# Ladme/groan_rs

Measured on AMD Instinct MI355X. Metric: frames/sec RMSD-fit, 1e6 atoms triclinic, 1/2/4/8 GPUs; HBM GB/s vs peak, higher is better.
Workload: dtype f32 (fp64 accumulators)

## Files before the change

### groan_rs_amd/csrc/gr_api.hip

```cpp
#include <hip/hip_runtime.h>

#include <cmath>
#include <cstdio>
#include <cstdlib>
#include <cstring>
#include <map>
#include <string>
#include <vector>

#include "../../include/groan_hip.h"
#include "gr_container.h"
#include "gr_kernels.h"
#include "gr_hot.h"
#include "gr_resident.h"
#include "gr_small.h"
#include "gr_xtc.h"
#include "gr_shape.h"
#include "gr_xtc_dev.h"
#include "gr_xtc_enc_dev.h"
#include "gr_trr.h"
#include "gr_cellgrid.h"
#include "gr_textio.h"
#include "gr_pool.h"
#include <set>
// ... 91 lines not shown
    uint32_t res_checkin = 0, res_closed = 0;
    uint32_t res_late_seen[2] = { 0, 0 };
    uint64_t res_lean_segments = 0, res_sync_fallbacks = 0;
    GrShapeSet *shape_set_dev = nullptr;
    unsigned long long *shape_mask_dev = nullptr, *shape_mask_host = nullptr; size_t shape_mask_cap = 0;
    uint32_t res_epoch = 0;
    bool res_in_use = false;
    uint64_t res_launches = 0, res_handshake_misses = 0, res_aborts = 0, res_redone_frames = 0;
    GrFrameState *state_dev = nullptr;
    GrFrameState *state_host = nullptr;
    GrFrameState *small_state = nullptr, *small_state_dev = nullptr;
    uint32_t *small_flag = nullptr, *small_flag_dev = nullptr;
    uint32_t small_seq = 0;
    uint32_t small_max = GR_SMALL_MAX_DEFAULT;
    uint64_t small_calls = 0, small_sync_fallbacks = 0;
    uint32_t *bad_dev = nullptr;
    uint32_t *bad_host = nullptr;
    float *pd_out = nullptr; size_t pd_cap = 0;
    hipEvent_t ev0 = nullptr, ev1 = nullptr;
    hipEvent_t pev[6 * GR_MAX_BATCH] = {};
    uint32_t sub_batch = 256;
    uint32_t chunks = 0;
    uint32_t fit_wgs = 0;
    int profile = 0;
    double prof_ms[4] = { 0, 0, 0, 0 };
    uint64_t prof_launches[4] = { 0, 0, 0, 0 };
    uint64_t prof_frames[4] = { 0, 0, 0, 0 };
    uint32_t n_cus = 0;
    unsigned char *xtc_host[2] = { nullptr, nullptr }, *xtc_dev[2] = { nullptr, nullptr }; size_t xtc_host_cap[2] = { 0, 0 }, xtc_dev_cap[2] = { 0, 0 };
    hipEvent_t xtc_ev[2] = { nullptr, nullptr };
    hipEvent_t xtc_unpacked[2] = { nullptr, nullptr };
    hipStream_t unpack_stream = nullptr;
    uint32_t xtc_bank = 0;
    float *wr_host = nullptr; size_t wr_cap = 0;
    void *xe_dev[6] = { nullptr, nullptr, nullptr, nullptr, nullptr, nullptr }; size_t xe_cap[6] = { 0, 0, 0, 0, 0, 0 };
    unsigned char *xe_host[2] = { nullptr, nullptr }; size_t xe_host_cap[2] = { 0, 0 };
    int xtc_dev_encode = 1;
    uint64_t xtc_dev_frames = 0;
    int strict = 0;
    gr_rmsd_plan *in_flight = nullptr;
    uint32_t in_flight_s0 = 0, in_flight_n = 0;
    uint64_t epoch = 1;
    std::string err;
    uint64_t err_index = 0;
    uint64_t counts[2] = { 0, 0 };
};

struct Pending {
    bool active = false, any_ok = false, consistent = true, fused = false, resident = false, rmsd_fast = false;
    uint32_t res_metro_ns = 0; bool res_metro_auto = false;
    uint32_t s0 = 0, nb = 0, n_prof_groups = 0, res_stream = 0, res_streams = 1;
    int fit = 0;
    std::vector<int> pre;
    std::vector<uint64_t> pre_idx;
    std::vector<std::string> pre_msg;
    GrSel sel = {};
    uint64_t group_n = 0;
    bool has_group = false;
    bool small = false; uint32_t small_seq = 0;
    uint32_t res_seq = 0, res_epoch = 0; bool res_fresh = false;
#ifdef GR_EXP_TIMELINE
    unsigned long long *tl_dev = nullptr;
#endif
};

struct gr_rmsd_plan {
    gr_ctx *target = nullptr;
    Pending pend;
    std::string group;
    uint64_t n_ref = 0;
    float *p_dev = nullptr, *w_dev = nullptr;
    float *p_span_dev = nullptr;
    std::vector<grc::Block> ref_blocks;
    bool span_ok = false;
    std::vector<float> w_host;
    GrPlanDev dev = {};
    int exact = 0;
    bool fit_behind_small = false;
    uint32_t last_fallbacks = 0;
    bool resolved = false;
    uint64_t resolved_epoch = 0;
};

namespace {

thread_local std::string g_create_err;

#define HIPCHK(ctx, call)                                                                      \
    do {                                                                                       \
        hipError_t e_ = (call);                                                                \
        if (e_ != hipSuccess) {                                                                \
            (ctx)->err = std::string(#call) + ": " + hipGetErrorString(e_);                    \
            return GR_E_HIP;                                                                   \
        }                                                                                      \
    } while (0)

int fail(gr_ctx *c, int status, const std::string &msg, uint64_t index = 0) {
    c->err = msg; c->err_index = index; return status;
}

GrSel make_sel(const Group &g) {
    GrSel s;
    s.n = (uint32_t)g.n; s.contiguous = g.contiguous ? 1u : 0u; s.start = g.start; s.g0 = g.start >> 8; s.idx = g.idx_dev;
    s.masked = (g.masked && g.mask_dev) ? (g.walk_rw ? 3u : 1u) : 0u; s.span = g.contiguous ? (uint32_t)g.n : g.span; s.mask = g.mask_dev;
    return s;
}

uint32_t chunks_for(const GrSel &s) {
// ... 275 lines not shown

int fetch_states(gr_ctx *c, uint32_t n) {
    HIPCHK(c, hipMemcpyAsync(c->state_host, c->state_dev, n * sizeof(GrFrameState), hipMemcpyDeviceToHost, c->stream));
    HIPCHK(c, hipStreamSynchronize(c->stream));
    return GR_OK;
}

int frame_status(gr_ctx *c, const GrFrameState &st) {
    if (st.status == GR_OK) return GR_OK;
    if (st.status == GR_E_NO_POSITION) return fail(c, GR_E_NO_POSITION, "atom has no position", st.err_index);
    if (st.status == GR_E_NO_MASS) return fail(c, GR_E_NO_MASS, "atom has no mass", st.err_index);
    return fail(c, st.status, "frame analysis failed");
}

static bool small_ok(const gr_ctx *c, const GrSel &sel) { return c->small_max != 0 && c->small_state != nullptr && sel.n <= c->small_max && !c->profile; }
static int small_wait(gr_ctx *c, uint32_t seq, uint32_t words = 1) {
    volatile uint32_t *w = c->small_flag;
    const auto t0 = std::chrono::steady_clock::now();
    for (uint32_t spins = 0; w[0] != seq || w[words - 1] != seq; ++spins) {
        if ((spins & 1023u) == 1023u && std::chrono::steady_clock::now() - t0 > std::chrono::milliseconds(20)) {
            c->small_sync_fallbacks++;
            HIPCHK(c, hipStreamSynchronize(c->stream));
            if (w[0] != seq || w[words - 1] != seq) return fail(c, GR_E_HIP, "a single-wave kernel ended without publishing its result");
            break;
        }
    }
    std::atomic_thread_fence(std::memory_order_acquire);
    c->small_calls++;
    return GR_OK;
}

static int res_next_epoch(gr_ctx *c, uint32_t *epoch) {
    if (++c->res_epoch == 0u) {
        HIPCHK(c, hipStreamSynchronize(c->stream));
        if (c->res_wgrec) HIPCHK(c, hipMemset(c->res_wgrec, 0, c->res_wgrec_cap * sizeof(unsigned long long)));
        HIPCHK(c, hipMemset(c->res_rec, 0, (size_t)GR_MAX_BATCH * 16 * sizeof(unsigned long long)));
        HIPCHK(c, hipMemset(c->res_abort + 2, 0, 2 * sizeof(uint32_t)));
        c->res_epoch = 1u;
    }
    *epoch = c->res_epoch;
    return GR_OK;
}
static int res_test_no_start(gr_ctx *c, uint32_t epoch) {
    if (!c->res_test_no_start) return GR_OK;
    const unsigned long long two = 2ull | ((unsigned long long)epoch << 32);
    c->res_test_no_start = 0;
    HIPCHK(c, hipMemcpyAsync(c->res_abort + 2, &two, sizeof two, hipMemcpyHostToDevice, c->stream));
    HIPCHK(c, hipStreamSynchronize(c->stream));
    return GR_OK;
}
template <int MODE>
static int res_close(gr_ctx *c, uint32_t nb, const double *fit_partials, uint32_t nparts, double sum_w, uint32_t epoch, bool fresh, uint32_t *seq) {
    const uint32_t sq = c->res_seq + 1u;
    k_res_close<MODE><<<dim3(nb), dim3(64), 0, c->stream>>>(fit_partials, nparts, sum_w, c->state_dev, c->res_rec, epoch, fresh ? 1u : 0u, c->res_abort, c->res_closed + nb,
                                                        c->res_out_dev->st, c->res_out_dev->words, &c->res_out_dev->seq, sq);
    HIPCHK(c, hipGetLastError());
    c->res_seq = sq; c->res_closed += nb; *seq = sq;
    return GR_OK;
}
static int res_collect(gr_ctx *c, uint32_t seq, uint32_t nb, uint32_t epoch, bool *started) {
    volatile uint32_t *w = &c->res_out->seq;
    const auto t0 = std::chrono::steady_clock::now();
    for (uint32_t spins = 0; *w != seq; ++spins) {
        if ((spins & 1023u) == 1023u && std::chrono::steady_clock::now() - t0 > std::chrono::milliseconds(20)) {
            c->res_sync_fallbacks++;
            HIPCHK(c, hipStreamSynchronize(c->stream));
            if (*w != seq) return fail(c, GR_E_HIP, "the kernel behind the resident pass ended without publishing its results");
            break;
        }
    }
    std::atomic_thread_fence(std::memory_order_acquire);
    memcpy(c->state_host, c->res_out->st, (size_t)nb * sizeof(GrFrameState));
    memcpy(c->res_words_host, c->res_out->words, 12 * sizeof(uint32_t));
    for (int k = 0; k < 2; ++k) { const uint32_t v = c->res_words_host[8 + k]; c->res_words_host[8 + k] = v - c->res_late_seen[k]; c->res_late_seen[k] = v; }
    *started = c->res_words_host[2] == 1u && c->res_words_host[3] == epoch;
    if (!*started || c->res_words_host[0]) HIPCHK(c, hipStreamSynchronize(c->stream));
    return GR_OK;
}

int center_stage(gr_ctx *c, uint32_t first_slot, uint32_t nf, const GrSel &sel, int kind, int weighted,
                 int mass_first, int target, int only_status = 0) {
    if (small_ok(c, sel)) {
        k_center_small_stage<<<dim3(nf), dim3(64), 0, c->stream>>>(c->frames, c->frame_stride, first_slot, c->masses, sel, c->boxes_dev, kind, weighted, mass_first, target, c->state_dev, only_status);
        HIPCHK(c, hipGetLastError());
        return GR_OK;
    }
    uint32_t nch = chunks_for(sel);
    if (nf > 1 && nch >= 8) nch &= ~7u;
    const dim3 grid(nch, nf), wg(GR_WG);
    if (kind == 0) k_center_sums<0><<<grid, wg, 0, c->stream>>>(c->frames, c->frame_stride, first_slot, c->masses, sel, c->boxes_dev, c->state_dev, weighted, c->cen_partials, only_status);
    else if (kind == 1) k_center_sums<1><<<grid, wg, 0, c->stream>>>(c->frames, c->frame_stride, first_slot, c->masses, sel, c->boxes_dev, c->state_dev, weighted, c->cen_partials, only_status);
    else k_center_sums<2><<<grid, wg, 0, c->stream>>>(c->frames, c->frame_stride, first_slot, c->masses, sel, c->boxes_dev, c->state_dev, weighted, c->cen_partials, only_status);
    k_center_finalize<<<dim3(nf), dim3(GR_WG), 0, c->stream>>>(c->cen_partials, nch, c->boxes_dev, first_slot, kind, weighted, mass_first, target, sel.n, c->state_dev, only_status);
    HIPCHK(c, hipGetLastError());
    return GR_OK;
}

int pbc_center_stages(gr_ctx *c, uint32_t first_slot, uint32_t nf, const GrSel &sel, int weighted, int only_status = 0) {
    if (small_ok(c, sel) && only_status == 0) {
        k_center_small_pbc<<<dim3(nf), dim3(64), 0, c->stream>>>(c->frames, c->frame_stride, first_slot, c->masses, sel, c->boxes_dev, weighted, c->state_dev);
        HIPCHK(c, hipGetLastError());
        return GR_OK;
    }
    int st = center_stage(c, first_slot, nf, sel, 1, 0, 0, 0, only_status);
    if (st != GR_OK) return st;
    return center_stage(c, first_slot, nf, sel, 2, weighted, 0, 1, only_status);
}

static bool center_onepass_ok(const gr_ctx *c, const GrSel &sel) {
    return c->com_onepass_min != 0 && (sel.contiguous || sel.masked) && sel.n >= c->com_onepass_min && c->two_pass;
// ... 1349 lines not shown
int gr_ctx_set_tuning(gr_ctx *c, int key, int64_t value) try {
    if (!c) return GR_E_INVALID_ARG;
    { int st = busy_check(c); if (st) return st; }
    switch (key) {
    case GR_TUNE_SUB_BATCH: if (value < 1 || value > GR_MAX_BATCH) break; c->sub_batch = (uint32_t)value; return GR_OK;
    case GR_TUNE_CHUNKS: if (value < 0 || value > GR_MAX_CHUNKS) break; c->chunks = (uint32_t)value; return GR_OK;
    case GR_TUNE_FIT_WGS: if (value < 0 || value > 65535) break; c->fit_wgs = (uint32_t)value; return GR_OK;
    case GR_TUNE_FUSE: c->fuse = value ? 1 : 0; return GR_OK;
    case GR_TUNE_SMALL_CALLS: if (value < 0 || value > 65536) break; c->small_max = (uint32_t)value; return GR_OK;
    case GR_TUNE_TWO_PASS: c->two_pass = value ? 1 : 0; return GR_OK;
    case GR_TUNE_RESIDENT: if (value < 0 || value > 2) break; c->resident = value; return GR_OK;
    case GR_TUNE_MASKED_SELECTIONS: if (value != 0 && value != 1) break; c->masked_sel = (int)value; return GR_OK;
    case GR_TUNE_XTC_DEVICE_ENCODE: if (value != 0 && value != 1) break; c->xtc_dev_encode = (int)value; return GR_OK;
    case GR_TUNE_RMSD_FAST: if (value != 0 && value != 1) break; c->rmsd_fast = (int)value; return GR_OK;
    case GR_TUNE_RMSD_FAST_MIN: if (value < 0 || value > 0x7fffffff) break; c->rmsd_fast_min = (uint32_t)value; return GR_OK;
    case GR_TUNE_RMSD_FAST_SIGMAS: if (value < 0 || value > 1000) break; c->rmsd_fast_sigmas = (int)value; return GR_OK;
    case GR_TUNE_PAIRDIST_SYMMETRIC: if (value != 0 && value != 1) break; c->pd_sym = (int)value; return GR_OK;
    case GR_TUNE_RESIDENT_WG_GROUPS: if (value != 0 && (value < 64 || value > GR_RES_GROUPS || value % 64 != 0)) break; c->res_wg_groups = (int)value; return GR_OK;
    case GR_TUNE_RESIDENT_STREAMS: if (value < 0 || value > GR_RES_MAX_STREAMS) break; c->res_streams = (int)value; return GR_OK;
    case GR_TUNE_RESIDENT_METRO_NS: if (value < 0 || value > 1000000 || (value > 1 && value < 100)) break; c->res_metro_ns = (int)value; c->metro = gr_ctx::Metro(); return GR_OK;
    case GR_TUNE_RESIDENT_FIT_LAST: if (value < 0 || value > 2) break; c->res_fit_last = (int)value; return GR_OK;
    case GR_TUNE_STREAM_WGS_PER_CU: if (value < 0 || value > 8) break; c->stream_wgs_cu = (int)value; return GR_OK;
    case GR_TUNE_CENTER_RESIDENT: if (value < 0 || value > 1) break; c->center_resident = (int)value; return GR_OK;
    case GR_TUNE_TRANSLATE_ROWS: if (value < 0 || value > 1) break; c->translate_rows = (int)value; return GR_OK;
    case GR_TUNE_RESIDENT_FILL: if (value < 1 || value > 16) break; c->res_fill16 = (int)value; return GR_OK;
    case GR_TUNE_RESIDENT_GROUPS: if (value != 2) break; return GR_OK;
    case GR_TUNE_TEST_RESIDENT_NO_START: c->res_test_no_start = value ? 1 : 0; return GR_OK;
    case GR_TUNE_TEST_RESIDENT_ABORT_AT: c->res_test_abort_at = value < 0 ? 0xFFFFFFFFu : (uint32_t)value; return GR_OK;
    default: break;
    }
    return fail(c, GR_E_INVALID_ARG, "unknown tuning key or value out of range");
} catch (...) { return gr_abi_guard(); }

static int rmsd_exact(gr_rmsd_plan *p, gr_ctx *c, const GrSel &sel, uint32_t first_slot, uint32_t nf, int fit) {
    int st = pbc_center_stages(c, first_slot, nf, sel, 1); if (st) return st;
    if (small_ok(c, sel)) {
        k_rmsd_small<1><<<dim3(nf), dim3(64), 0, c->stream>>>(c->frames, c->frame_stride, first_slot, c->masses, sel, c->boxes_dev, p->dev, c->state_dev, 1, nullptr, nullptr, 0u);
    } else {
        const uint32_t nch = chunks_for(sel);
        k_rmsd_accum<1><<<dim3(nch, nf), dim3(GR_WG), 0, c->stream>>>(c->frames, c->frame_stride, first_slot, c->masses, sel, c->boxes_dev, p->dev, c->state_dev, c->acc_partials);
        k_rmsd_finalize<1><<<dim3(nf), dim3(GR_WG), 0, c->stream>>>(c->acc_partials, nch, c->frames, c->frame_stride, first_slot, sel, c->boxes_dev, p->dev, c->state_dev);
    }
    if (fit) {
        const uint32_t gx = (uint32_t)std::min<uint64_t>(((c->n >> 2) + GR_WG * 4 - 1) / (GR_WG * 4) + 1, 1024);
        k_fit_pk<false><<<dim3(gx, nf), dim3(GR_WG), 0, c->stream>>>(c->frames, c->frame_stride, first_slot, (uint32_t)c->n, c->boxes_dev, p->dev, c->state_dev, c->masses, sel, nullptr);
    }
    HIPCHK(c, hipGetLastError());
    return GR_OK;
}

static int segment_begin(gr_rmsd_plan *p, uint32_t s0, uint32_t nb, int fit) {
    gr_ctx *c = p->target;
    Pending &q = p->pend;
    q = Pending();
    q.s0 = s0; q.nb = nb; q.fit = fit; q.active = true;
    SlotUse use(c, s0, nb);
    const Group *g = find_group(c, p->group.c_str());
    q.pre.assign(nb, GR_OK); q.pre_idx.assign(nb, 0); q.pre_msg.assign(nb, std::string());
    for (uint32_t f = 0; f < nb; ++f) {
        int s = box_check(c, s0 + f);
        if (s == GR_OK && !g) s = fail(c, GR_E_GROUP_NOT_FOUND, p->group);
        if (s == GR_OK && g->n == 0) s = fail(c, GR_E_EMPTY_GROUP, p->group);
        q.pre[f] = s;
        if (s != GR_OK) { q.pre_msg[f] = c->err; q.pre_idx[f] = c->err_index; }
        q.any_ok = q.any_ok || s == GR_OK;
    }
    if (!q.any_ok) return GR_OK;
    const GrSel sel = make_sel(*g);
    q.sel = sel; q.group_n = g->n; q.has_group = true;
    if (!p->resolved || p->resolved_epoch != c->epoch) {
        p->resolved_epoch = c->epoch;
        bool same = (g->n == p->n_ref);
        if (same) { size_t k = 0; for (uint64_t i : grc::expand(g->blocks)) { const float a = c->masses_host[i], b = p->w_host[k++]; if (!(a == b)) { same = false; break; } } }
        p->dev.w_is_mass = same ? 1u : 0u; p->resolved = true;
        p->span_ok = p->p_span_dev != nullptr && g->masked && g->mask_dev != nullptr && g->blocks == p->ref_blocks;
    }
    q.consistent = (g->n == p->n_ref);
    const bool fast_asked = c->two_pass && c->rmsd_fast && p->dev.w_is_mass != 0 && g->n >= c->rmsd_fast_min && ((!fit && sel.contiguous) || (sel.masked && p->span_ok));
    const bool small = q.consistent && !p->exact && small_ok(c, sel) && !fast_asked;
    if (small && nb == 1) {
        q.small = true; q.small_seq = ++c->small_seq;
        k_rmsd_small<0><<<dim3(1), dim3(64), 0, c->stream>>>(c->frames, c->frame_stride, s0, c->masses, sel, c->boxes_dev, p->dev,
                                                         c->state_dev, 0, c->small_state_dev, c->small_flag_dev, q.small_seq);
        if (fit) k_fit_pk<false><<<dim3(fit_grid(c, 1), 1), dim3(GR_WG), 0, c->stream>>>(c->frames, c->frame_stride, s0, (uint32_t)c->n, c->boxes_dev, p->dev, c->state_dev, c->masses, sel, nullptr);
        p->fit_behind_small = fit != 0;
        HIPCHK(c, hipGetLastError());
        return GR_OK;
    }
    bool states_unset = false;
    {
        bool all_ok = true;
        for (uint32_t f = 0; f < nb; ++f) all_ok = all_ok && q.pre[f] == GR_OK;
        states_unset = all_ok;
        if (!all_ok) {
            for (uint32_t f = 0; f < nb; ++f) { GrFrameState z = {}; z.err_index = GR_NOIDX; z.status = q.pre[f]; c->state_host[f] = z; }
            HIPCHK(c, hipMemcpyAsync(c->state_dev, c->state_host, nb * sizeof(GrFrameState), hipMemcpyHostToDevice, c->stream));
        }
    }
    auto zero_states = [&]() -> int { if (!states_unset) return GR_OK; states_unset = false; return state_reset(c, nb); };
    int st;
    if (!(q.consistent && !p->exact && !small)) { st = zero_states(); if (st) return st; }
    if (small) {
        k_rmsd_small<0><<<dim3(nb), dim3(64), 0, c->stream>>>(c->frames, c->frame_stride, s0, c->masses, sel, c->boxes_dev, p->dev, c->state_dev, 1, nullptr, nullptr, 0u);
        if (fit) k_fit_pk<false><<<dim3(fit_grid(c, nb), nb), dim3(GR_WG), 0, c->stream>>>(c->frames, c->frame_stride, s0, (uint32_t)c->n, c->boxes_dev, p->dev, c->state_dev, c->masses, sel, nullptr);
        HIPCHK(c, hipGetLastError());
    } else if (!q.consistent) {
        st = pbc_center_stages(c, s0, nb, sel, 1); if (st) return st;
    } else if (p->exact) {
        st = rmsd_exact(p, c, sel, s0, nb, fit); if (st) return st;
    } else {
        const uint32_t sb = c->sub_batch;
        const bool lite = fit && sel.contiguous && c->two_pass;
        const bool msk = sel.masked && p->span_ok;
        const bool fast = c->two_pass && c->rmsd_fast && p->dev.w_is_mass != 0 && g->n >= c->rmsd_fast_min && ((!fit && sel.contiguous) || msk);
        q.rmsd_fast = fast;
        p->dev.fast_sigmas = (float)c->rmsd_fast_sigmas;
        GrPlanDev plan_span = p->dev; plan_span.p = p->p_span_dev;
        const uint32_t n_groups = (nb + sb - 1) / sb;
        if (lite) {
            size_t need = 0;
            for (uint32_t f0 = 0; f0 < nb; f0 += sb) need = std::max(need, (size_t)nb * fit_grid(c, std::min<uint32_t>(sb, nb - f0)) * (GR_WG / 64));
            if (need > c->fit_partials_cap) {
                if (c->fit_partials) (void)hipFree(c->fit_partials);
                c->fit_partials = nullptr; c->fit_partials_cap = 0;
                HIPCHK(c, hipMalloc(&c->fit_partials, need * sizeof(double)));
                c->fit_partials_cap = need;
            }
        }
        const bool fused = (lite || fast) && c->fuse;
        q.fused = fused;
        hipStream_t S = c->stream;
        uint32_t res_streams = 1, res_gwg = GR_RES_GROUPS;
        const bool res_msk = fit && msk && c->two_pass && p->dev.w_is_mass != 0;
        uint32_t res_wgs = resident_wgs(c, lite || res_msk, nb, sel, &res_streams, &res_gwg);
        if (res_wgs && !resident_acquire(c->device)) res_wgs = 0;
        if (res_wgs) c->res_in_use = true;
        if (res_wgs) {
            const uint32_t res_stream = res_wgs * res_streams;
            const uint32_t n_fin = std::min<uint32_t>(res_streams > 8 ? GR_RES_MAX_FIN : 8, c->res_max_wgs - res_stream);
            if ((size_t)nb * res_wgs * GrResShape::WAVES > c->fit_partials_cap) {
                if (c->fit_partials) (void)hipFree(c->fit_partials);
                c->fit_partials = nullptr; c->fit_partials_cap = 0;
                HIPCHK(c, hipMalloc(&c->fit_partials, (size_t)nb * res_wgs * GrResShape::WAVES * sizeof(double)));
                c->fit_partials_cap = (size_t)nb * res_wgs * GrResShape::WAVES;
            }
            const size_t rec_words = (size_t)nb * ((res_wgs + GR_RES_REC_PAD - 1u) & ~(uint32_t)(GR_RES_REC_PAD - 1u)) * GR_RES_REC_WORDS;
            if (rec_words > c->res_wgrec_cap) {
                if (c->res_wgrec) (void)hipFree(c->res_wgrec);
                c->res_wgrec = nullptr; c->res_wgrec_cap = 0;
                HIPCHK(c, hipMalloc(&c->res_wgrec, rec_words * sizeof(unsigned long long)));
                HIPCHK(c, hipMemsetAsync(c->res_wgrec, 0, rec_words * sizeof(unsigned long long), S));
                c->res_wgrec_cap = rec_words;
            }
            GrResCtl ctl;
            st = res_next_epoch(c, &ctl.epoch); if (st) return st;
            ctl.wgrec = c->res_wgrec; ctl.rec = c->res_rec; ctl.abort = c->res_abort; ctl.progress = c->res_progress; ctl.n_stream = res_stream; ctl.n_fin = n_fin;
            ctl.checkin_target = c->res_checkin + res_stream + n_fin; ctl.fresh_states = states_unset ? 1u : 0u;
            ctl.wgs_frame = res_wgs; ctl.streams = res_streams; ctl.groups_wg = res_gwg;
            ctl.team_waves = resident_team_waves(res_wgs, res_streams);
            ctl.patience_ticks = (unsigned long long)c->wall_khz * 3000ull; ctl.start_ticks = (unsigned long long)c->wall_khz * 200ull;
            ctl.test_abort_frame = c->res_test_abort_at; c->res_test_abort_at = 0xFFFFFFFFu;
            {
                const uint64_t shape = ((uint64_t)res_wgs << 40) ^ ((uint64_t)res_streams << 32) ^ ((uint64_t)res_gwg << 16) ^ (uint64_t)(c->n & 0xFFFF) ^ ((uint64_t)(sel.start == 0 && sel.n == c->n) << 63);
                uint32_t period_ns = 0;
                q.res_metro_auto = false;
                if (c->res_metro_ns >= 100) period_ns = (uint32_t)c->res_metro_ns;
                else if (c->res_metro_ns == 0) {
                    gr_ctx::Metro &m = c->metro;
                    if (m.shape != shape) { m = gr_ctx::Metro(); m.shape = shape; }
                    if (m.off_for) m.off_for--;
                    else if (m.free_ns > 0) period_ns = (uint32_t)(m.T_ns + 0.5);
                    q.res_metro_auto = true;
                }
                q.res_metro_ns = period_ns;
                ctl.metro_t16 = (uint32_t)std::min<uint64_t>(0xFFFFFFFFull, (uint64_t)period_ns * (uint64_t)c->wall_khz * 16ull / 1000000ull);
                ctl.metro_lead = (uint32_t)((uint64_t)c->wall_khz * 2000ull / 1000000ull);
            }
#ifdef GR_EXP_STEPTIME
            {
                static unsigned long long *dbg_dev = nullptr;
                if (!dbg_dev) (void)hipMalloc(&dbg_dev, (size_t)GR_MAX_CHUNKS * 8 * 4 * sizeof(unsigned long long));
                ctl.dbg = getenv("GR_STEPTIME") ? dbg_dev : nullptr;
                g_steptime_dbg = ctl.dbg;
            }
#endif
#ifdef GR_EXP_TIMELINE
            {
                static unsigned long long *tl_dev = nullptr; static size_t tl_cap = 0;
                if (nb > tl_cap) { if (tl_dev) (void)hipFree(tl_dev); tl_dev = nullptr; tl_cap = 0; if (hipMalloc(&tl_dev, (size_t)nb * 8 * sizeof(unsigned long long)) == hipSuccess) tl_cap = nb; }
                ctl.tl = getenv("GR_TIMELINE") ? tl_dev : nullptr;
                if (ctl.tl) HIPCHK(c, hipMemsetAsync(ctl.tl, 0, (size_t)nb * 8 * sizeof(unsigned long long), S));
                q.tl_dev = ctl.tl;
            }
#endif
            float *frames = c->frames; size_t stride = c->frame_stride; uint32_t slot0 = s0, nfr = nb, natoms = (uint32_t)c->n;
            const float *masses = c->masses; GrSel sel_arg = sel; const GrBox *boxes = c->boxes_dev; GrPlanDev plan = res_msk ? plan_span : p->dev;
            GrFrameState *states = c->state_dev; double *fparts = c->fit_partials;
            void *args[] = { &frames, &stride, &slot0, &nfr, &natoms, &masses, &sel_arg, &boxes, &plan, &states, &fparts, &ctl };
            bool ubox = true;
            for (uint32_t f = 1; f < nb && ubox; ++f) ubox = memcmp(&c->boxes_host[s0 + f], &c->boxes_host[s0], sizeof(GrBox)) == 0;
#ifdef GR_EXP_NO_UBOX
            ubox = false;
#endif
            const bool whole = sel.start == 0 && sel.n == c->n;
            const bool fit_last = c->res_fit_last ? c->res_fit_last == 2 : (uint64_t)res_stream * 10u >= (uint64_t)c->res_max_wgs * 9u;
            const void *fn = resident_fn(p->dev.w_is_mass != 0, ubox, whole, fit_last);
            const uint32_t lanes = GrResShape::LANES, lds = GrResShape::LDS_BYTES;
            st = res_test_no_start(c, ctl.epoch); if (st) return st;
            if (c->profile) EVREC(c, c->pev[0], true, S);
            const hipError_t le = hipLaunchKernel(fn, dim3(res_stream + n_fin), dim3(lanes), args, lds, S);
            if (le == hipSuccess) {
                if (c->profile) EVREC(c, c->pev[1], true, S);
                c->res_checkin += res_stream + n_fin;
                q.res_fresh = states_unset; q.res_epoch = ctl.epoch;
                states_unset = false;
                st = res_close<0>(c, nb, c->fit_partials, res_wgs * GrResShape::WAVES, p->dev.sw, ctl.epoch, q.res_fresh, &q.res_seq); if (st) return st;
                q.resident = true; q.res_stream = res_stream; q.res_streams = res_streams;
                q.rmsd_fast = false;
                c->res_last_streams = res_streams;
            } else {
                (void)hipGetLastError();
                c->res_max_wgs = 0;
                resident_done(c);
            }
        }
        if (!q.resident) { st = zero_states(); if (st) return st; }
        for (uint32_t g = 0; g < n_groups && !q.resident; ++g) {
            const uint32_t f0 = g * sb, nf = std::min<uint32_t>(sb, nb - f0), nch = batch_chunks(c, sel, nf), gx = fit_grid(c, nf);
            GrAccPartial *parts = c->acc_partials + (size_t)f0 * GR_MAX_CHUNKS;
            if (c->profile) EVREC(c, c->pev[6 * g], true, S);
            if (lite) k_sums_pk<false><<<dim3(nch, nf), dim3(GR_WG), 0, S>>>(c->frames, c->frame_stride, s0 + f0, c->masses, sel, c->boxes_dev, p->dev, parts,
                                                                             fused ? c->fuse_cnt + f0 : nullptr, c->state_dev + f0);
            else if (fast && msk) k_sums_pk<false, true, true><<<dim3(nch, nf), dim3(GR_WG), 0, S>>>(c->frames, c->frame_stride, s0 + f0, c->masses, sel, c->boxes_dev, plan_span, parts,
                                                                                                      fused ? c->fuse_cnt + f0 : nullptr, c->state_dev + f0);
            else if (fast) k_sums_pk<false, true><<<dim3(nch, nf), dim3(GR_WG), 0, S>>>(c->frames, c->frame_stride, s0 + f0, c->masses, sel, c->boxes_dev, p->dev, parts,
                                                                                        fused ? c->fuse_cnt + f0 : nullptr, c->state_dev + f0);
            else k_rmsd_accum<0><<<dim3(nch, nf), dim3(GR_WG), 0, S>>>(c->frames, c->frame_stride, s0 + f0, c->masses, sel, c->boxes_dev, p->dev, c->state_dev + f0, parts);
            if (c->profile) EVREC(c, c->pev[6 * g + 1], true, S);
            if (!fused) {
                if (c->profile) EVREC(c, c->pev[6 * g + 2], true, S);
                if (lite) k_rmsd_finalize_lite<false><<<dim3(nf), dim3(64), 0, S>>>(parts, nch, c->frames, c->frame_stride, s0 + f0, sel, c->boxes_dev, p->dev, c->state_dev + f0);
                else if (fast) k_rmsd_finalize_lite<false, true><<<dim3(nf), dim3(64), 0, S>>>(parts, nch, c->frames, c->frame_stride, s0 + f0, sel, c->boxes_dev, msk ? plan_span : p->dev, c->state_dev + f0);
                else k_rmsd_finalize<0><<<dim3(nf), dim3(GR_WG), 0, S>>>(parts, nch, c->frames, c->frame_stride, s0 + f0, sel, c->boxes_dev, p->dev, c->state_dev + f0);
                if (c->profile) EVREC(c, c->pev[6 * g + 3], true, S);
            }
            if (fit) {
                if (c->profile) EVREC(c, c->pev[6 * g + 4], true, S);
                if (lite) k_fit_pk<true><<<dim3(gx, nf), dim3(GR_WG), stream_lds(c, GR_STREAM_WGS_CU_DEFAULT), S>>>(c->frames, c->frame_stride, s0 + f0, (uint32_t)c->n, c->boxes_dev, p->dev, c->state_dev + f0, c->masses, sel, c->fit_partials + (size_t)f0 * gx * (GR_WG / 64));
                else k_fit_pk<false><<<dim3(gx, nf), dim3(GR_WG), 0, S>>>(c->frames, c->frame_stride, s0 + f0, (uint32_t)c->n, c->boxes_dev, p->dev, c->state_dev + f0, c->masses, sel, nullptr);
                if (c->profile) EVREC(c, c->pev[6 * g + 5], true, S);
                if (lite) k_rmsd_close<<<dim3(nf), dim3(64), 0, S>>>(c->fit_partials + (size_t)f0 * gx * (GR_WG / 64), gx * (GR_WG / 64), p->dev.sw, c->state_dev + f0);
            }
        }
        HIPCHK(c, hipGetLastError());
        if (c->profile) q.n_prof_groups = q.resident ? 0 : n_groups;
    }
    if (!q.resident) HIPCHK(c, hipMemcpyAsync(c->state_host, c->state_dev, nb * sizeof(GrFrameState), hipMemcpyDeviceToHost, c->stream));
    return GR_OK;
}

static int segment_end(gr_rmsd_plan *p, float *rmsd_out, int *status_out, float *R_out, std::vector<GrFrameState> *final_states = nullptr) {
    gr_ctx *c = p->target;
    Pending &q = p->pend;
    if (!q.active) return fail(c, GR_E_INVALID_ARG, "no batch in flight");
    q.active = false;
    const uint32_t nb = q.nb, s0 = q.s0;
    const int fit = q.fit;
    int first_err = GR_OK; uint64_t first_err_index = 0; std::string first_err_msg; uint64_t first_counts[2] = { 0, 0 };
    auto note = [&](int s) { if (s != GR_OK && first_err == GR_OK) { first_err = s; first_err_index = c->err_index; first_err_msg = c->err; first_counts[0] = c->counts[0]; first_counts[1] = c->counts[1]; } };
    if (!q.any_ok) {
        for (uint32_t f = 0; f < nb; ++f) {
            c->err = q.pre_msg[f]; c->err_index = q.pre_idx[f]; note(q.pre[f]);
            if (status_out) status_out[f] = q.pre[f];
            if (rmsd_out) rmsd_out[f] = NAN;
            if (R_out) for (int k = 0; k < 9; ++k) R_out[9 * (size_t)f + k] = NAN;
        }
        if (final_states) { final_states->assign(nb, GrFrameState{}); for (uint32_t f = 0; f < nb; ++f) { (*final_states)[f].status = q.pre[f]; (*final_states)[f].err_index = GR_NOIDX; } }
    } else {
        if (!q.has_group) return fail(c, GR_E_INVALID_ARG, "batch state lost");
        const GrSel sel = q.sel;
        bool res_started = false;
        if (q.small) { const int sw = small_wait(c, q.small_seq); if (sw) return sw; c->state_host[0] = *c->small_state; }
        else if (q.resident) { const int sw = res_collect(c, q.res_seq, nb, q.res_epoch, &res_started); if (sw) { resident_done(c); return sw; } }
        else HIPCHK(c, hipStreamSynchronize(c->stream));
        std::vector<uint8_t> redo;
        std::vector<uint8_t> torn;
#ifdef GR_EXP_TIMELINE
        if (q.resident && q.tl_dev) {
            std::vector<unsigned long long> tl((size_t)nb * 8);
            if (hipMemcpy(tl.data(), q.tl_dev, tl.size() * sizeof(unsigned long long), hipMemcpyDeviceToHost) == hipSuccess) {
                double sum[8] = { 0 }; double period = 0; uint64_t n = 0, polled = 0, fpolls = 0; unsigned long long prev = 0;
                for (uint32_t f = 0; f < nb; ++f) {
                    const unsigned long long *t = &tl[(size_t)f * 8];
                    if (!t[0] || !t[1] || !t[5] || !(t[6] & 0xFFFFFFFFFFFFull)) continue;
                    const unsigned long long look = t[6] & 0xFFFFFFFFFFFFull;
                    sum[0] += (double)((long long)(t[1] - t[0])); sum[1] += (double)((long long)(t[2] - t[1])); sum[2] += (double)((long long)(t[3] - t[2]));
                    sum[3] += (double)((long long)(t[4] - t[3])); sum[4] += (double)((long long)(t[5] - t[4])); sum[5] += (double)((long long)(look - t[5]));
                    sum[6] += (double)((long long)(look - t[0]));
                    if (prev) period += (double)((long long)(t[0] - prev));
                    prev = t[0];
                    polled += (t[6] >> 48) != 0; fpolls += t[7]; n++;
                }
                if (n > 1) fprintf(stderr, "timeline (%llu frames, us): pub->all records %.2f | ->team totals %.2f | state load %.2f | closing %.2f | publish+store %.2f | ->wg0 looks %.2f | pub->look %.2f | period %.3f | wg0 polled for %.0f %% of the frames | finalizer polls per frame %.1f\n",
                                   (unsigned long long)n, sum[0] / n / 100.0, sum[1] / n / 100.0, sum[2] / n / 100.0, sum[3] / n / 100.0, sum[4] / n / 100.0, sum[5] / n / 100.0, sum[6] / n / 100.0,
                                   period / (n - 1) / 100.0, 100.0 * polled / n, (double)fpolls / n);
            }
        }
#endif
        if (q.resident) {
            resident_done(c);
            if (!res_started) {
                c->res_handshake_misses++;
                c->res_backoff = c->res_backoff ? std::min<uint32_t>(c->res_backoff * 2u, 1024u) : 4u;
                c->res_skip = c->res_backoff + 1u;
                const int fit_again = q.fit;
                const uint32_t s0_again = q.s0, nb_again = q.nb;
                int st2 = segment_begin(p, s0_again, nb_again, fit_again);
                if (st2) { p->pend.active = false; resident_done(c); return st2; }
                return segment_end(p, rmsd_out, status_out, R_out, final_states);
            }
            c->res_backoff = 0;
            if (q.res_fresh) c->res_lean_segments++;
            const uint32_t aborted = c->res_words_host[0];
            if (aborted) {
                (void)hipMemset(c->res_abort, 0, sizeof(uint32_t));
// ... 131 lines not shown
                std::vector<GrFrameState> fs2;
                Pending sub;
                std::swap(sub, p->pend);
                st_redo = segment_begin(p, s0 + f0, f1 - f0, fit);
                if (st_redo == GR_OK) {
                    const int st_nested = segment_end(p, nullptr, nullptr, nullptr, &fs2);
                    if (fs2.size() != (size_t)(f1 - f0)) st_redo = st_nested != GR_OK ? st_nested : GR_E_HIP;
                    else for (uint32_t f = f0; f < f1; ++f) res[f] = fs2[f - f0];
                } else { p->pend.active = false; resident_done(c); }
                std::swap(sub, p->pend);
                c->res_redone_frames += f1 - f0;
                f0 = f1;
            }
            c->resident = keep;
            if (st_redo != GR_OK) return st_redo;
        }
        if (q.rmsd_fast) {
            for (uint32_t f0 = 0; f0 < nb; ) {
                if (res[f0].status != GR_ST_REDO_EXACT) { if (q.pre[f0] == GR_OK) c->rmsd_fast_frames++; ++f0; continue; }
                uint32_t f1 = f0;
                while (f1 < nb && res[f1].status == GR_ST_REDO_EXACT) ++f1;
                const uint32_t nf = f1 - f0, nch = batch_chunks(c, sel, nf);
                SlotUse use(c, s0 + f0, nf);
                int st = state_reset(c, nf); if (st) return st;
                GrAccPartial *parts = c->acc_partials;
                k_rmsd_accum<0><<<dim3(nch, nf), dim3(GR_WG), 0, c->stream>>>(c->frames, c->frame_stride, s0 + f0, c->masses, sel, c->boxes_dev, p->dev, c->state_dev, parts);
                k_rmsd_finalize<0><<<dim3(nf), dim3(GR_WG), 0, c->stream>>>(parts, nch, c->frames, c->frame_stride, s0 + f0, sel, c->boxes_dev, p->dev, c->state_dev);
                if (fit) {
                    const uint32_t gx = fit_grid(c, nf);
                    k_fit_pk<false><<<dim3(gx, nf), dim3(GR_WG), 0, c->stream>>>(c->frames, c->frame_stride, s0 + f0, (uint32_t)c->n, c->boxes_dev, p->dev, c->state_dev, c->masses, sel, nullptr);
                }
                HIPCHK(c, hipGetLastError());
                st = fetch_states(c, nf); if (st) return st;
                for (uint32_t f = f0; f < f1; ++f) res[f] = c->state_host[f - f0];
                c->rmsd_exact_redos += nf;
                f0 = f1;
            }
        }
        for (uint32_t f0 = 0; f0 < nb; ) {
            if (res[f0].status != GR_ST_FALLBACK || (!redo.empty() && redo[f0])) { ++f0; continue; }
            uint32_t f1 = f0;
            while (f1 < nb && res[f1].status == GR_ST_FALLBACK && (redo.empty() || !redo[f1])) ++f1;
            const uint32_t nf = f1 - f0;
            p->last_fallbacks += nf;
            SlotUse use(c, s0 + f0, nf);
            int st = state_reset(c, nf); if (st) return st;
            st = rmsd_exact(p, c, sel, s0 + f0, nf, fit); if (st) return st;
            st = fetch_states(c, nf); if (st) return st;
            for (uint32_t f = f0; f < f1; ++f) res[f] = c->state_host[f - f0];
            f0 = f1;
        }
        for (uint32_t f = 0; f < nb; ++f) {
            int s = res[f].status;
            if (q.pre[f] != GR_OK) { s = q.pre[f]; c->err = q.pre_msg[f]; c->err_index = q.pre_idx[f]; }
            else if (!torn.empty() && torn[f]) s = fail(c, GR_E_HIP, "the resident RMSD-fit pass stalled while this frame was being fitted: some of its atoms carry the fitted coordinates, others the original ones (frame index in gr_last_error_index)", f);
            else if (s == GR_OK && !q.consistent) {
                c->counts[0] = p->n_ref; c->counts[1] = q.group_n;
                s = fail(c, GR_E_INCONSISTENT_GROUP, p->group);
            } else if (s != GR_OK) {
                s = frame_status(c, res[f]);
            }
            note(s);
            if (status_out) status_out[f] = s;
            if (rmsd_out) rmsd_out[f] = (s == GR_OK) ? res[f].rmsd : NAN;
            if (R_out) for (int k = 0; k < 9; ++k) R_out[9 * (size_t)f + k] = (s == GR_OK) ? res[f].R[k] : NAN;
        }
        if (final_states) *final_states = res;
    }
    if (first_err != GR_OK) { c->err = first_err_msg; c->err_index = first_err_index; c->counts[0] = first_counts[0]; c->counts[1] = first_counts[1]; }
    return first_err;
}

static int rmsd_batch_impl(gr_rmsd_plan *p, uint32_t first_slot, uint32_t n_frames, float *rmsd_out, int *status_out, float *R_out, int fit) {
    if (!p || !p->target) return GR_E_INVALID_ARG;
    gr_ctx *c = p->target;
    int st = slot_check(c, first_slot, n_frames); if (st) return st;
    (void)hipSetDevice(c->device);
    if (p->pend.active) return fail(c, GR_E_INVALID_ARG, "a batch begun with gr_rmsd_batch_begin is still in flight");
    p->last_fallbacks = 0;
    int first_err = GR_OK; uint64_t e_idx = 0; std::string e_msg; uint64_t e_cnt[2] = { 0, 0 };
    for (uint32_t b0 = 0; b0 < n_frames; b0 += GR_MAX_BATCH) {
        const uint32_t nb = std::min<uint32_t>(GR_MAX_BATCH, n_frames - b0);
        st = segment_begin(p, first_slot + b0, nb, fit);
        if (st) { p->pend.active = false; resident_done(c); return st; }
        st = segment_end(p, rmsd_out ? rmsd_out + b0 : nullptr, status_out ? status_out + b0 : nullptr, R_out ? R_out + 9 * (size_t)b0 : nullptr);
        if (st == GR_E_HIP) return st;
        if (st != GR_OK && first_err == GR_OK) { first_err = st; e_idx = c->err_index; e_msg = c->err; e_cnt[0] = c->counts[0]; e_cnt[1] = c->counts[1]; }
    }
    if (first_err != GR_OK) { c->err = e_msg; c->err_index = e_idx; c->counts[0] = e_cnt[0]; c->counts[1] = e_cnt[1]; }
    return first_err;
}

int gr_rmsd_batch_begin(gr_rmsd_plan *p, uint32_t first_slot, uint32_t n, int fit) try {
    if (!p || !p->target) return GR_E_INVALID_ARG;
    gr_ctx *c = p->target;
    int st = slot_check(c, first_slot, n); if (st) return st;
    if (n > GR_MAX_BATCH) return fail(c, GR_E_INVALID_ARG, "at most 1024 frames per asynchronous batch");
    if (p->pend.active) return fail(c, GR_E_INVALID_ARG, "a batch is already in flight on this plan");
    (void)hipSetDevice(c->device);
    p->last_fallbacks = 0;
    st = segment_begin(p, first_slot, n, fit ? 1 : 0);
    if (st) { p->pend.active = false; resident_done(c); } else { c->in_flight = p; c->in_flight_s0 = first_slot; c->in_flight_n = n; }
    return st;
} catch (...) { return gr_abi_guard(); }
int gr_rmsd_batch_end(gr_rmsd_plan *p, float *rmsd_out, int *status_out, float *R_out) try {
    if (!p || !p->target) return GR_E_INVALID_ARG;
    (void)hipSetDevice(p->target->device);
// ... 970 lines not shown
```

### groan_rs_amd/csrc/gr_resident.h

```cpp
#pragma once
#include <type_traits>
#include "gr_hot.h"

struct GrResShape {
    static constexpr int LANES = 512, WAVES = LANES / 64;
#ifndef GR_RES_K
#define GR_RES_K 6
#endif
    static constexpr int K = GR_RES_K;
    static constexpr int R = 8;
    static constexpr int PARK_F4 = K * 3 * LANES;
    static constexpr int WSUM_F = R * WAVES * 32;
#ifdef GR_EXP_TIMELINE
    static constexpr int TL_BYTES = 128 * 4 * 8;
#else
    static constexpr int TL_BYTES = 0;
#endif
    static constexpr int LDS_BYTES = PARK_F4 * 16 + WSUM_F * 4 + R * WAVES * 8 + 3 * R * 4 + 2 * WAVES * 4 + TL_BYTES;
    static constexpr int REC_PER_WAVE = 256 / WAVES, LANES_PER_REC = 64 / REC_PER_WAVE, WORDS_PER_LANE = 32 / LANES_PER_REC;
};
#ifndef GR_RES_SLEEP
#define GR_RES_SLEEP 2
#endif
#ifndef GR_RES_BAL
// ... 892 lines not shown
        request(i + 1, nxt);
#endif
        if (i < n_turns) {
            if (MODE == 1) sums_cen(i, cur, Bs);
            else if (V) sums(i, cur, Bs, va, vb);
            lds_put(ps, va);
            if (ps == 0u) { Q0 = vb; asm volatile("; set 0 in"); } else if (ps == 1u) { Q1 = vb; asm volatile("; set 1 in"); } else if (ps == 2u) { Q2 = vb; asm volatile("; set 2 in"); }
            else if (ps == 3u) { Q3 = vb; asm volatile("; set 3 in"); } else if (ps == 4u) { Q4 = vb; asm volatile("; set 4 in"); } else { Q5 = vb; asm volatile("; set 5 in"); }
            if (!V && MODE != 1) sums(i, cur, Bs, va, vb);
        }
#if GR_RES_LATE_COMBINE
        if (i == n_turns && n_turns > 0u && claim(n_turns - 1u)) { if constexpr (MODE == 1) combine_cen(n_turns - 1u); else combine_rmsd(n_turns - 1u); }
#endif
    };
    auto step = [&](uint32_t i, Landing &cur, Landing &nxt) { if constexpr (FL) step_sums_first(i, cur, nxt); else step_fit_first(i, cur, nxt); };
    for (uint32_t i = 0; i < n_iter && !bail; i += 2) {
        step(i, L0, L1);
        if (!bail && i + 1 < n_iter) step(i + 1, L1, L0);
    }
    if (lane == 0) {
        ctl.progress[wg_all * WAVES + wave] = n_fitted;
        (void)__hip_atomic_fetch_max(reinterpret_cast<unsigned long long *>(ctl.abort + 6), (unsigned long long)wall_clock64(), __ATOMIC_RELAXED, __HIP_MEMORY_SCOPE_AGENT);
        if (n_late) (void)__hip_atomic_fetch_add(ctl.abort + 8, n_late, __ATOMIC_RELAXED, __HIP_MEMORY_SCOPE_AGENT);
        if (n_waited) (void)__hip_atomic_fetch_add(ctl.abort + 9, n_waited, __ATOMIC_RELAXED, __HIP_MEMORY_SCOPE_AGENT);
#ifdef GR_EXP_STEPTIME
        if (ctl.dbg) {
            unsigned long long *o = ctl.dbg + (size_t)(wg_all * WAVES + wave) * 4u;
            unsigned long long tot = 0; for (int k = 0; k < 7; ++k) tot += st_acc[k];
            o[0] = st_acc[4]; o[1] = st_acc[7] | (st_combines << 32);
            o[2] = (__builtin_amdgcn_s_getreg((20 << 0) | (0 << 6) | (3 << 11)) & 7u) | (simd_of[wave] << 8);
            o[3] = tot;
        }
        if ((wg_all == 0u || wg_all == ctl.n_stream / 2u) && (wave == 0u || wave == 5u)) {
            unsigned long long *o = reinterpret_cast<unsigned long long *>(ctl.abort + 16) + ((wg_all ? 2u : 0u) + (wave ? 1u : 0u)) * 8u;
            for (int k = 0; k < 8; ++k) o[k] = st_acc[k];
        }
#endif
        if (clk_wave) {
            const unsigned long long dc = (unsigned long long)clock64() - clk_c0, dw = (unsigned long long)wall_clock64() - clk_w0;
            gr_st_agent(ctl.abort + 10, (uint32_t)(dc >> 8)); gr_st_agent(ctl.abort + 11, (uint32_t)(dw >> 8));
        }
    }
#ifdef GR_EXP_TIMELINE
    if (tl_wg && wave == 0 && !bail) {
        for (uint32_t t = (n_turns > 128u ? n_turns - 128u : 0u) + lane; t < n_turns; t += 64u) {
            const size_t f = kf(t);
            ctl.tl[f * 8 + 0] = tls[(t & 127u) * 4u + 0u];
            ctl.tl[f * 8 + 6] = tls[(t & 127u) * 4u + 1u] | (tls[(t & 127u) * 4u + 2u] << 48);
        }
    }
#endif
}

template <int MODE>
__global__ __launch_bounds__(64) void k_res_close(const double *__restrict__ fit_partials, uint32_t nparts, double sum_w, GrFrameState *state,
                                                  const unsigned long long *__restrict__ rec, uint32_t epoch, uint32_t fresh_states, uint32_t *ctl_words,
                                                  uint32_t done_target, GrFrameState *out_states, uint32_t *out_words, uint32_t *out_seq, uint32_t seq) {
    constexpr uint32_t NW = sizeof(GrFrameState) / 4u, W_RMSD = offsetof(GrFrameState, rmsd) / 4u, W_STATUS = offsetof(GrFrameState, status) / 4u;
    static_assert(sizeof(GrFrameState) % 4u == 0 && NW <= 64u, "a frame state is exported by one wave, a word per lane");
    const uint32_t frame = blockIdx.x, lane = threadIdx.x;
    uint32_t *sw = reinterpret_cast<uint32_t *>(state + frame);
    uint32_t w = 0u;
    if (fresh_states && (uint32_t)(gr_ld_agent(rec + (size_t)frame * 16u) >> 32) != epoch) {
        GrFrameState z = {};
        z.err_index = GR_NOIDX; z.status = GR_ST_ABORTED;
        if (lane < NW) { w = reinterpret_cast<const uint32_t *>(&z)[lane]; sw[lane] = w; }
    } else if (lane < NW) w = sw[lane];
    const int status = __shfl((int)w, (int)W_STATUS, 64);
    if (MODE == 0 && status == 0) {
        double s0 = 0.0, s1 = 0.0, s2 = 0.0, s3 = 0.0;
        const double *p = fit_partials + (size_t)frame * nparts;
        uint32_t k = lane;
        for (; k + 192 < nparts; k += 256) { s0 += p[k]; s1 += p[k + 64]; s2 += p[k + 128]; s3 += p[k + 192]; }
        for (; k < nparts; k += 64) s0 += p[k];
        const double s = gr_wave_sum((s0 + s1) + (s2 + s3));
        float r = 0.0f;
        if (lane == 0) { r = (float)sqrt(fmax(s, 0.0) / sum_w); state[frame].rmsd = r; }
        r = __shfl(r, 0, 64);
        if (lane == W_RMSD) w = __float_as_uint(r);
    }
    if (lane < NW) reinterpret_cast<uint32_t *>(out_states + frame)[lane] = w;
    __threadfence_system();
    uint32_t n = 0u;
    if (lane == 0) n = __hip_atomic_fetch_add(ctl_words + 12, 1u, __ATOMIC_ACQ_REL, __HIP_MEMORY_SCOPE_AGENT) + 1u;
    n = (uint32_t)__builtin_amdgcn_readfirstlane((int)n);
    if (n != done_target) return;
    if (lane < 12u) out_words[lane] = gr_ld_agent(ctl_words + lane);
    __threadfence_system();
    if (lane == 0) __hip_atomic_store(out_seq, seq, __ATOMIC_RELEASE, __HIP_MEMORY_SCOPE_SYSTEM);
}
```

Baseline: 140,600.

## Pack eight frames per close workgroup and trim per-segment host bookkeeping

The resident close kernel now handles eight frames per workgroup, one wave per frame. Only wave 0 of each workgroup does the system fence and the completion-counter atomic, so there are fewer system-scope fences and atomics per segment. Host-side setup reuses the Pending vectors, records only the frames that failed, and computes the same-box and all-ok flags in the existing check loop. The cost is a block-wide barrier and explicit waitcnts, plus a lower_bound lookup when reporting per-frame errors.

```diff
diff --git a/groan_rs_amd/csrc/gr_api.hip b/groan_rs_amd/csrc/gr_api.hip
--- a/groan_rs_amd/csrc/gr_api.hip
+++ b/groan_rs_amd/csrc/gr_api.hip
@@ -167,8 +167,15 @@
     uint32_t s0 = 0, nb = 0, n_prof_groups = 0, res_stream = 0, res_streams = 1;
     int fit = 0;
     std::vector<int> pre;
-    std::vector<uint64_t> pre_idx;
-    std::vector<std::string> pre_msg;
+    struct PreFail { uint32_t frame; uint64_t index; std::string msg; };
+    std::vector<PreFail> pre_fail;
+    const PreFail &failed(uint32_t f) const { return *std::lower_bound(pre_fail.begin(), pre_fail.end(), f, [](const PreFail &a, uint32_t b) { return a.frame < b; }); }
+    void restart() {
+        std::vector<int> a; std::vector<PreFail> b;
+        a.swap(pre); b.swap(pre_fail); b.clear();
+        *this = Pending();
+        a.swap(pre); b.swap(pre_fail);
+    }
     GrSel sel = {};
     uint64_t group_n = 0;
     bool has_group = false;
@@ -550,10 +557,11 @@
 template <int MODE>
 static int res_close(gr_ctx *c, uint32_t nb, const double *fit_partials, uint32_t nparts, double sum_w, uint32_t epoch, bool fresh, uint32_t *seq) {
     const uint32_t sq = c->res_seq + 1u;
-    k_res_close<MODE><<<dim3(nb), dim3(64), 0, c->stream>>>(fit_partials, nparts, sum_w, c->state_dev, c->res_rec, epoch, fresh ? 1u : 0u, c->res_abort, c->res_closed + nb,
-                                                        c->res_out_dev->st, c->res_out_dev->words, &c->res_out_dev->seq, sq);
+    const uint32_t wgs = (nb + GR_RES_CLOSE_WAVES - 1u) / GR_RES_CLOSE_WAVES;
+    k_res_close<MODE><<<dim3(wgs), dim3(GR_RES_CLOSE_WAVES * 64), 0, c->stream>>>(fit_partials, nparts, sum_w, c->state_dev, c->res_rec, epoch, fresh ? 1u : 0u, nb, c->res_abort,
+                                                                              c->res_closed + wgs, c->res_out_dev->st, c->res_out_dev->words, &c->res_out_dev->seq, sq);
     HIPCHK(c, hipGetLastError());
-    c->res_seq = sq; c->res_closed += nb; *seq = sq;
+    c->res_seq = sq; c->res_closed += wgs; *seq = sq;
     return GR_OK;
 }
 static int res_collect(gr_ctx *c, uint32_t seq, uint32_t nb, uint32_t epoch, bool *started) {
@@ -2009,18 +2017,20 @@
 static int segment_begin(gr_rmsd_plan *p, uint32_t s0, uint32_t nb, int fit) {
     gr_ctx *c = p->target;
     Pending &q = p->pend;
-    q = Pending();
+    q.restart();
     q.s0 = s0; q.nb = nb; q.fit = fit; q.active = true;
     SlotUse use(c, s0, nb);
     const Group *g = find_group(c, p->group.c_str());
-    q.pre.assign(nb, GR_OK); q.pre_idx.assign(nb, 0); q.pre_msg.assign(nb, std::string());
+    bool all_ok = true, same_box = true;
+    q.pre.resize(nb);
     for (uint32_t f = 0; f < nb; ++f) {
         int s = box_check(c, s0 + f);
         if (s == GR_OK && !g) s = fail(c, GR_E_GROUP_NOT_FOUND, p->group);
         if (s == GR_OK && g->n == 0) s = fail(c, GR_E_EMPTY_GROUP, p->group);
         q.pre[f] = s;
-        if (s != GR_OK) { q.pre_msg[f] = c->err; q.pre_idx[f] = c->err_index; }
-        q.any_ok = q.any_ok || s == GR_OK;
+        if (s != GR_OK) { all_ok = false; q.pre_fail.push_back({ f, c->err_index, c->err }); }
+        else q.any_ok = true;
+        same_box = same_box && memcmp(&c->boxes_host[s0 + f], &c->boxes_host[s0], sizeof(GrBox)) == 0;
     }
     if (!q.any_ok) return GR_OK;
     const GrSel sel = make_sel(*g);
@@ -2046,8 +2056,6 @@
     }
     bool states_unset = false;
     {
-        bool all_ok = true;
-        for (uint32_t f = 0; f < nb; ++f) all_ok = all_ok && q.pre[f] == GR_OK;
         states_unset = all_ok;
         if (!all_ok) {
             for (uint32_t f = 0; f < nb; ++f) { GrFrameState z = {}; z.err_index = GR_NOIDX; z.status = q.pre[f]; c->state_host[f] = z; }
@@ -2154,8 +2162,7 @@
             const float *masses = c->masses; GrSel sel_arg = sel; const GrBox *boxes = c->boxes_dev; GrPlanDev plan = res_msk ? plan_span : p->dev;
             GrFrameState *states = c->state_dev; double *fparts = c->fit_partials;
             void *args[] = { &frames, &stride, &slot0, &nfr, &natoms, &masses, &sel_arg, &boxes, &plan, &states, &fparts, &ctl };
-            bool ubox = true;
-            for (uint32_t f = 1; f < nb && ubox; ++f) ubox = memcmp(&c->boxes_host[s0 + f], &c->boxes_host[s0], sizeof(GrBox)) == 0;
+            bool ubox = same_box;
 #ifdef GR_EXP_NO_UBOX
             ubox = false;
 #endif
@@ -2227,7 +2234,8 @@
     auto note = [&](int s) { if (s != GR_OK && first_err == GR_OK) { first_err = s; first_err_index = c->err_index; first_err_msg = c->err; first_counts[0] = c->counts[0]; first_counts[1] = c->counts[1]; } };
     if (!q.any_ok) {
         for (uint32_t f = 0; f < nb; ++f) {
-            c->err = q.pre_msg[f]; c->err_index = q.pre_idx[f]; note(q.pre[f]);
+            if (q.pre[f] != GR_OK) { const Pending::PreFail &e = q.failed(f); c->err = e.msg; c->err_index = e.index; }
+            note(q.pre[f]);
             if (status_out) status_out[f] = q.pre[f];
             if (rmsd_out) rmsd_out[f] = NAN;
             if (R_out) for (int k = 0; k < 9; ++k) R_out[9 * (size_t)f + k] = NAN;
@@ -2465,7 +2473,7 @@
         }
         for (uint32_t f = 0; f < nb; ++f) {
             int s = res[f].status;
-            if (q.pre[f] != GR_OK) { s = q.pre[f]; c->err = q.pre_msg[f]; c->err_index = q.pre_idx[f]; }
+            if (q.pre[f] != GR_OK) { const Pending::PreFail &e = q.failed(f); s = q.pre[f]; c->err = e.msg; c->err_index = e.index; }
             else if (!torn.empty() && torn[f]) s = fail(c, GR_E_HIP, "the resident RMSD-fit pass stalled while this frame was being fitted: some of its atoms carry the fitted coordinates, others the original ones (frame index in gr_last_error_index)", f);
             else if (s == GR_OK && !q.consistent) {
                 c->counts[0] = p->n_ref; c->counts[1] = q.group_n;
diff --git a/groan_rs_amd/csrc/gr_resident.h b/groan_rs_amd/csrc/gr_resident.h
--- a/groan_rs_amd/csrc/gr_resident.h
+++ b/groan_rs_amd/csrc/gr_resident.h
@@ -968,40 +968,48 @@
 #endif
 }
 
+#define GR_RES_CLOSE_WAVES 8
 template <int MODE>
-__global__ __launch_bounds__(64) void k_res_close(const double *__restrict__ fit_partials, uint32_t nparts, double sum_w, GrFrameState *state,
-                                                  const unsigned long long *__restrict__ rec, uint32_t epoch, uint32_t fresh_states, uint32_t *ctl_words,
+__global__ __launch_bounds__(GR_RES_CLOSE_WAVES * 64) void k_res_close(const double *__restrict__ fit_partials, uint32_t nparts, double sum_w, GrFrameState *state,
+                                                  const unsigned long long *__restrict__ rec, uint32_t epoch, uint32_t fresh_states, uint32_t nb, uint32_t *ctl_words,
                                                   uint32_t done_target, GrFrameState *out_states, uint32_t *out_words, uint32_t *out_seq, uint32_t seq) {
-    constexpr uint32_t NW = sizeof(GrFrameState) / 4u, W_RMSD = offsetof(GrFrameState, rmsd) / 4u, W_STATUS = offsetof(GrFrameState, status) / 4u;
+    constexpr uint32_t NW = sizeof(GrFrameState) / 4u, W_RMSD = offsetof(GrFrameState, rmsd) / 4u, W_STATUS = offsetof(GrFrameState, status) / 4u,
+                       W_ERR_INDEX = offsetof(GrFrameState, err_index) / 4u;
     static_assert(sizeof(GrFrameState) % 4u == 0 && NW <= 64u, "a frame state is exported by one wave, a word per lane");
-    const uint32_t frame = blockIdx.x, lane = threadIdx.x;
-    uint32_t *sw = reinterpret_cast<uint32_t *>(state + frame);
-    uint32_t w = 0u;
-    if (fresh_states && (uint32_t)(gr_ld_agent(rec + (size_t)frame * 16u) >> 32) != epoch) {
-        GrFrameState z = {};
-        z.err_index = GR_NOIDX; z.status = GR_ST_ABORTED;
-        if (lane < NW) { w = reinterpret_cast<const uint32_t *>(&z)[lane]; sw[lane] = w; }
-    } else if (lane < NW) w = sw[lane];
-    const int status = __shfl((int)w, (int)W_STATUS, 64);
-    if (MODE == 0 && status == 0) {
-        double s0 = 0.0, s1 = 0.0, s2 = 0.0, s3 = 0.0;
-        const double *p = fit_partials + (size_t)frame * nparts;
-        uint32_t k = lane;
-        for (; k + 192 < nparts; k += 256) { s0 += p[k]; s1 += p[k + 64]; s2 += p[k + 128]; s3 += p[k + 192]; }
-        for (; k < nparts; k += 64) s0 += p[k];
-        const double s = gr_wave_sum((s0 + s1) + (s2 + s3));
-        float r = 0.0f;
-        if (lane == 0) { r = (float)sqrt(fmax(s, 0.0) / sum_w); state[frame].rmsd = r; }
-        r = __shfl(r, 0, 64);
-        if (lane == W_RMSD) w = __float_as_uint(r);
+    const uint32_t wave = (uint32_t)__builtin_amdgcn_readfirstlane((int)(threadIdx.x >> 6)), lane = threadIdx.x & 63u;
+    const uint32_t frame = blockIdx.x * GR_RES_CLOSE_WAVES + wave;
+    if (frame < nb) {
+        uint32_t *sw = reinterpret_cast<uint32_t *>(state + frame);
+        uint32_t w = 0u;
+        if (fresh_states && (uint32_t)(gr_ld_agent(rec + (size_t)frame * 16u) >> 32) != epoch) {
+            if (lane < NW) { w = lane == W_STATUS ? (uint32_t)GR_ST_ABORTED : lane == W_ERR_INDEX ? GR_NOIDX : 0u; sw[lane] = w; }
+        } else if (lane < NW) w = sw[lane];
+        const int status = __shfl((int)w, (int)W_STATUS, 64);
+        if (MODE == 0 && status == 0) {
+            double s0 = 0.0, s1 = 0.0, s2 = 0.0, s3 = 0.0;
+            const double *p = fit_partials + (size_t)frame * nparts;
+            uint32_t k = lane;
+            for (; k + 192 < nparts; k += 256) { s0 += p[k]; s1 += p[k + 64]; s2 += p[k + 128]; s3 += p[k + 192]; }
+            for (; k < nparts; k += 64) s0 += p[k];
+            const double s = gr_wave_sum((s0 + s1) + (s2 + s3));
+            float r = 0.0f;
+            if (lane == 0) { r = (float)sqrt(fmax(s, 0.0) / sum_w); state[frame].rmsd = r; }
+            r = __shfl(r, 0, 64);
+            if (lane == W_RMSD) w = __float_as_uint(r);
+        }
+        if (lane < NW) __hip_atomic_store(reinterpret_cast<uint32_t *>(out_states + frame) + lane, w, __ATOMIC_RELAXED, __HIP_MEMORY_SCOPE_SYSTEM);
     }
-    if (lane < NW) reinterpret_cast<uint32_t *>(out_states + frame)[lane] = w;
+    asm volatile("s_waitcnt vmcnt(0)" ::: "memory");
+    __syncthreads();
+    if (wave != 0u) return;
     __threadfence_system();
+    asm volatile("s_waitcnt vmcnt(0)" ::: "memory");
     uint32_t n = 0u;
     if (lane == 0) n = __hip_atomic_fetch_add(ctl_words + 12, 1u, __ATOMIC_ACQ_REL, __HIP_MEMORY_SCOPE_AGENT) + 1u;
     n = (uint32_t)__builtin_amdgcn_readfirstlane((int)n);
     if (n != done_target) return;
-    if (lane < 12u) out_words[lane] = gr_ld_agent(ctl_words + lane);
+    if (lane < 12u) __hip_atomic_store(out_words + lane, gr_ld_agent(ctl_words + lane), __ATOMIC_RELAXED, __HIP_MEMORY_SCOPE_SYSTEM);
     __threadfence_system();
+    asm volatile("s_waitcnt vmcnt(0)" ::: "memory");
     if (lane == 0) __hip_atomic_store(out_seq, seq, __ATOMIC_RELEASE, __HIP_MEMORY_SCOPE_SYSTEM);
 }
```

After: 140,500. About the same (-0.1%).
